# zivy/LSQRRecipes

Hardware: AMD Instinct MI355X
Metric: RANSAC hypotheses/sec + final-fit residual, 10M pts, 1/2/4/8 GPU (higher is better)
Workload: dtype f64; 1 GPU; PlaneParametersEstimator + RANSAC, 10000000 points, 50% outliers, delta=0.50 (BASELINE.json configs[1]); points=10000000, streams=4, world_size=1, collectives=none (single GPU), repeats=3

## Files before the change

### include/lsqr_hip.h

```cpp
#ifndef LSQR_HIP_H
#define LSQR_HIP_H

#include <stddef.h>
#include <stdint.h>

#ifdef __cplusplus
extern "C" {
#endif

#if defined(__GNUC__)
#define LSQR_API __attribute__((visibility("default")))
#else
#define LSQR_API
#endif

typedef enum {
  LSQR_OK = 0,
  LSQR_EMPTY = 1,
  LSQR_ERR_INVALID = 2,
  LSQR_ERR_NO_DEVICE = 3,
  LSQR_ERR_HIP = 4,
  LSQR_ERR_STATE = 5
} lsqr_status;

// ... 218 lines not shown
LSQR_API int lsqr_multi_upload(lsqr_multi *m, const void *host_records, size_t count, size_t stride_bytes);
LSQR_API int lsqr_multi_batch_fit(lsqr_multi *m, uint64_t seed, uint64_t first_index, size_t H_per_device,
                                  double *params_out, uint8_t *consensus_out, lsqr_ransac_info *info);
LSQR_API int lsqr_multi_ransac(lsqr_multi *m, double p, uint64_t seed, double *params_out,
                               uint8_t *consensus_out, lsqr_ransac_info *info);

LSQR_API int lsqr_ransac_exhaustive(lsqr_ctx *ctx, double *params_out, uint8_t *consensus_out,
                                    lsqr_ransac_info *info);
LSQR_API int lsqr_replay_init(size_t n, int k, double p, uint64_t state[6]);
LSQR_API size_t lsqr_replay(size_t n, int k, double p, const uint32_t *subsets,
                            const uint8_t *valid, const uint32_t *votes, size_t H,
                            uint64_t base_index, void *dedup_set, uint64_t state[6]);
LSQR_API void *lsqr_dedup_create(int k);
LSQR_API void lsqr_dedup_destroy(void *set);

LSQR_API int lsqr_set_option(lsqr_ctx *ctx, const char *name, int value);

LSQR_API int lsqr_index_info(const lsqr_ctx *ctx, uint64_t out[4]);

LSQR_API int lsqr_scan_workload(lsqr_ctx *ctx, uint32_t *bound_out, uint64_t out[8]);

LSQR_API int lsqr_scan_work(lsqr_ctx *ctx, uint64_t out[8]);

LSQR_API int lsqr_lm_persist_info(const lsqr_ctx *ctx, uint64_t out[8], uint64_t *trace, uint32_t trace_cap,
                                  uint32_t *trace_n);

LSQR_API int lsqr_profile_enable(lsqr_ctx *ctx, int on);
LSQR_API int lsqr_profile_get(lsqr_ctx *ctx, int kernel_id, uint64_t *launches, double *total_ms);
LSQR_API int lsqr_profile_reset(lsqr_ctx *ctx);

#ifdef __cplusplus
}
#endif
#endif
```

### lsqrrecipes_amd/_lib.py

```python
import ctypes as C
import os

import numpy as np

_HERE = os.path.dirname(os.path.abspath(__file__))
LIB_PATH = os.path.join(_HERE, "liblsqr_hip.so")

OK, EMPTY, ERR_INVALID, ERR_NO_DEVICE, ERR_HIP, ERR_STATE = range(6)
PLANE, SPHERE, LINE, DENSE, US_SINGLE, US_POINTER, ABSOR, PIVOT, RAY, LINE2D, PHANTOM = 1, 2, 3, 4, 5, 6, 7, 8, 9, 10, 11
LS_ALGEBRAIC, LS_GEOMETRIC = 0, 1
LS_ANALYTIC, LS_ITERATIVE = 0, 1
KERNEL_IDS = {"sample": 0, "estimate": 1, "scan": 2, "mask": 3, "moments": 4, "solve": 5,
              "index": 6, "absmax": 7}


class LsqrError(RuntimeError):
    def __init__(self, status, msg):
        RuntimeError.__init__(self, "lsqr_hip status %d: %s" % (status, msg))
        self.status = status


class ModelCfg(C.Structure):
    _fields_ = [("model", C.c_int32), ("dim", C.c_int32), ("delta", C.c_double),
                ("ls_type", C.c_int32), ("reserved", C.c_int32), ("aux", C.c_double)]
# ... 110 lines not shown
    "lsqr_batch_fit_wait": (C.c_int, [_ctx, C.c_int, C.c_void_p, C.POINTER(RansacInfo)]),
    "lsqr_multi_create": (C.c_int, [C.POINTER(C.c_int), C.c_int, C.POINTER(C.c_void_p)]),
    "lsqr_multi_destroy": (None, [C.c_void_p]),
    "lsqr_multi_size": (C.c_int, [C.c_void_p]),
    "lsqr_multi_transport": (C.c_char_p, [C.c_void_p, C.POINTER(C.c_double)]),
    "lsqr_multi_ctx": (C.c_void_p, [C.c_void_p, C.c_int]),
    "lsqr_multi_last_error": (C.c_char_p, [C.c_void_p]),
    "lsqr_multi_set_model": (C.c_int, [C.c_void_p, C.POINTER(ModelCfg)]),
    "lsqr_multi_upload": (C.c_int, [C.c_void_p, C.c_void_p, C.c_size_t, C.c_size_t]),
    "lsqr_multi_batch_fit": (C.c_int, [C.c_void_p, C.c_uint64, C.c_uint64, C.c_size_t, C.c_void_p, C.c_void_p,
                                       C.POINTER(RansacInfo)]),
    "lsqr_multi_ransac": (C.c_int, [C.c_void_p, C.c_double, C.c_uint64, C.c_void_p, C.c_void_p,
                                    C.POINTER(RansacInfo)]),
    "lsqr_ransac_exhaustive": (C.c_int, [_ctx, C.c_void_p, C.c_void_p, C.POINTER(RansacInfo)]),
    "lsqr_replay_init": (C.c_int, [C.c_size_t, C.c_int, C.c_double, _u64p]),
    "lsqr_replay": (C.c_size_t, [C.c_size_t, C.c_int, C.c_double, C.c_void_p, C.c_void_p,
                                 C.c_void_p, C.c_size_t, C.c_uint64, C.c_void_p, _u64p]),
    "lsqr_dedup_create": (C.c_void_p, [C.c_int]),
    "lsqr_dedup_destroy": (None, [C.c_void_p]),
    "lsqr_set_option": (C.c_int, [_ctx, C.c_char_p, C.c_int]),
    "lsqr_index_info": (C.c_int, [_ctx, _u64p]),
    "lsqr_scan_workload": (C.c_int, [_ctx, C.c_void_p, _u64p]),
    "lsqr_scan_work": (C.c_int, [_ctx, _u64p]),
    "lsqr_lm_persist_info": (C.c_int, [_ctx, _u64p, _u64p, C.c_uint32, C.POINTER(C.c_uint32)]),
    "lsqr_profile_enable": (C.c_int, [_ctx, C.c_int]),
    "lsqr_profile_get": (C.c_int, [_ctx, C.c_int, _u64p, _dp]),
    "lsqr_profile_reset": (C.c_int, [_ctx]),
}

_lib = None


def load():
    global _lib
    if _lib is None:
        if not os.path.exists(LIB_PATH):
            raise LsqrError(ERR_NO_DEVICE, "%s not built: run `python -c 'import __graft_entry__ as"
                            " g; g.build()'` or make -C lsqrrecipes_amd/csrc" % LIB_PATH)
        lib = C.CDLL(LIB_PATH)
        for name, (res, args) in SIGNATURES.items():
            fn = getattr(lib, name)
            fn.restype = res
            fn.argtypes = args
        _lib = lib
    return _lib

# ... 10 lines not shown
```

### lsqrrecipes_amd/context.py

```python
import ctypes as C

import numpy as np

from . import _lib as L


class Context:
    def __init__(self, device=0):
        self._lib = L.load()
        h = C.c_void_p()
        st = self._lib.lsqr_ctx_create(int(device), C.byref(h))
        if st != L.OK:
            raise L.LsqrError(st, "lsqr_ctx_create(device=%d): %s" % (
                device, self._lib.lsqr_status_string(st).decode()))
        self._h = h
        self.device = device
        self.cfg = None
        self._keep = None

    def close(self):
        if getattr(self, "_h", None):
            self._lib.lsqr_ctx_destroy(self._h)
            self._h = None

# ... 663 lines not shown
        self._chk(self._lib.lsqr_index_info(self._h, out))
        return {"built": bool(out[0]), "observations": int(out[1]), "cells": int(out[2]),
                "cell_points": int(out[3])}

    def scan_workload(self, want_bounds=False):
        H = self._lib.lsqr_num_hypotheses(self._h)
        ub = np.zeros(H, dtype=np.uint32) if want_bounds else None
        out = (C.c_uint64 * 8)()
        self._chk(self._lib.lsqr_scan_workload(self._h, L.ptr(ub), out))
        r = {"pairs": int(out[0]), "level1_evaluations": int(out[1]), "cells": int(out[2]),
             "cell_points": int(out[3]), "bounded": bool(out[4]), "pilots": int(out[5]),
             "second_pass": int(out[6]), "pairs_counted": int(out[7])}
        if want_bounds:
            r["bounds"] = ub
        return r

    def scan_work(self):
        out = (C.c_uint64 * 8)()
        self._chk(self._lib.lsqr_scan_work(self._h, out))
        return {"early_exit": bool(out[0]), "row_hypothesis_pairs": int(out[1]), "row_hypothesis_pairs_all": int(out[2]),
                "candidates": int(out[3]), "dropped_first": int(out[4]), "alive_at_end": int(out[5]),
                "ambiguous_pairs": int(out[6]), "band_records": int(out[7])}

    def synchronize(self):
        self._chk(self._lib.lsqr_synchronize(self._h))


class MultiContext:

    def __init__(self, devices):
        self._lib = L.load()
        arr = (C.c_int * len(devices))(*[int(d) for d in devices])
        h = C.c_void_p()
        st = self._lib.lsqr_multi_create(arr, len(devices), C.byref(h))
        if st != L.OK:
            raise L.LsqrError(st, "lsqr_multi_create(%s): %s" % (list(devices), self._lib.lsqr_status_string(st).decode()))
        self._h = h
        self.size = len(devices)
        self.cfg = None

    def close(self):
        if getattr(self, "_h", None):
            self._lib.lsqr_multi_destroy(self._h)
            self._h = None

    __del__ = close
# ... 91 lines not shown
```

### lsqrrecipes_amd/csrc/axis.h

```cpp
#pragma once
#include <hip/hip_runtime.h>
#include <stdint.h>

#include "cells.h"

namespace lsqr {

struct CellAxis {
  float e[3];
  float tmax;
};
constexpr int kAxisGroup = 8;

template <int NPT>
__global__ __launch_bounds__(256) void k_cell_moments(const double *__restrict__ sorted, size_t ns, uint32_t ncells,
                                                      const CellBox *__restrict__ boxes, double *__restrict__ mom) {
  const uint32_t cell = blockIdx.x * 4 + (threadIdx.x >> 6);
  if (cell >= ncells) return;
  const int lane = threadIdx.x & 63;
  constexpr uint32_t CP = 64 * NPT;
  const CellBox bx = boxes[cell];
  double s[10] = {0, 0, 0, 0, 0, 0, 0, 0, 0, 0};
  for (int k = 0; k < NPT; k++) {
    const size_t i = (size_t)cell * CP + k * 64 + lane;
// ... 124 lines not shown
  bool ok[NPT];
#pragma unroll
  for (int k = 0; k < NPT; k++) {
    const unsigned long long v = s[k * 64 + lane];
    const uint32_t src = (uint32_t)(v & 0xFFFFFFFFu), key = (uint32_t)(v >> 32);
    ok[k] = key != 0xFFFFFFFFu;
    const size_t i = (size_t)cell * CP + (ok[k] ? src : 0);
    const size_t ic = i < ns ? i : 0;
    px[k] = sorted[ic * 3], py[k] = sorted[ic * 3 + 1], pz[k] = sorted[ic * 3 + 2];
    uint32_t u = key;
    u ^= (u >> 31) ? 0x80000000u : 0xFFFFFFFFu;
    tv[k] = ok[k] ? __builtin_bit_cast(float, u) : __builtin_inff();
  }
  asm volatile("s_waitcnt vmcnt(0)" ::: "memory");
  __syncthreads();
  if (!live) return;
#pragma unroll
  for (int k = 0; k < NPT; k++) {
    const size_t i = (size_t)cell * CP + k * 64 + lane;
    cellT[i] = tv[k];
    if (ok[k] && i < ns) sorted[i * 3] = px[k], sorted[i * 3 + 1] = py[k], sorted[i * 3 + 2] = pz[k];
  }
  if (lane == 0) axis[cell].tmax = tmax;
}

template <int PP>
__global__ __launch_bounds__(512) void k_bound_axis(const CellBox *__restrict__ boxes, const CellAxis *__restrict__ axis,
                                                    const float *__restrict__ cellT, size_t ns, uint32_t ncells,
                                                    const float *__restrict__ rows, uint32_t H,
                                                    const uint32_t *__restrict__ h_dev, CellConsts cc, float thr_up,
                                                    float thr_dn, float xabs, uint32_t cells_per_block,
                                                    uint32_t *__restrict__ ub, uint32_t *__restrict__ lb) {
  typedef PlaneCell<3> CM;
  constexpr uint32_t CP = 128 * PP;
  constexpr int ROW = CM::ROW, NR4 = ROW / 4;
  const int lane = threadIdx.x & 63;
  if (h_dev) {
    const uint32_t hd = *h_dev;
    H = hd < H ? hd : H;
  }
  const uint32_t grp = blockIdx.y * 8 + (threadIdx.x >> 6);
  const uint32_t h = grp * 64 + lane;
  if (blockIdx.y * 512 >= H) return;
  const bool active = h - lane < H;
  float row[ROW];
  {
// ... 184 lines not shown
```

### lsqrrecipes_amd/csrc/cells.h

```cpp
#pragma once
#include <hip/hip_runtime.h>
#include <stdint.h>

#include "models.h"

#pragma clang diagnostic ignored "-Winline-asm"

namespace lsqr {

constexpr int kCellPtsMin = 128;
constexpr uint32_t kGroupPad = 4, kCellPad = 16;
constexpr uint32_t kBlockPad = 6;
constexpr uint32_t kQueues = 32;
constexpr uint32_t kQueuePitch = 1088;

struct CellBox {
  float c[3];
  float h[3];
  float pad[2];
};

__device__ inline unsigned long long ord_u64(double v) {
  unsigned long long b;
  __builtin_memcpy(&b, &v, 8);
  return (b >> 63) ? ~b : (b | 0x8000000000000000ULL);
}
inline double ord_u64_inv(unsigned long long o) {
  unsigned long long b = (o >> 63) ? (o & 0x7FFFFFFFFFFFFFFFULL) : ~o;
  double v;
  memcpy(&v, &b, 8);
  return v;
}

struct BoundsRow {
  unsigned long long mn[3], mx[3], amax, nonfinite;
};
template <int D>
__global__ __launch_bounds__(256) void k_bounds(const double *__restrict__ data, size_t stride,
                                                size_t n, BoundsRow *__restrict__ rows) {
  unsigned long long mn[D], mx[D], am = 0, bad = 0;
  for (int d = 0; d < D; d++) mn[d] = ~0ULL, mx[d] = 0ULL;
  auto one = [&](const double(&x)[D]) {
// ... 539 lines not shown
      sb.c[d] = cf;
      sb.h[d] = (!nan && hd <= 3.4e38) ? f32_up(hd) : 3.4028234e38f;
      r2 += (double)sb.h[d] * (double)sb.h[d];
    } else {
      sb.c[d] = 0.0f;
      sb.h[d] = 0.0f;
    }
  }
  const double rad = sqrt(r2) * (1.0 + 1e-6);
  sb.pad[0] = rad <= 3.4e38 ? f32_up(rad) : 3.4028234e38f;
  sb.pad[1] = 0.0f;
  sboxes[sc] = sb;
}

struct CellConsts {
  float f[8];
};
template <class CM>
constexpr bool cell_prepared() {
  if constexpr (requires { CM::PREPARED; }) return CM::PREPARED != 0;
  return false;
}
template <class CM>
struct HypWords {
  static_assert(sizeof(typename CM::Hyp) % 16 == 0, "a prepared Hyp is padded to a multiple of 16 bytes");
  enum { N4 = sizeof(typename CM::Hyp) / 16 };
  float w[4 * N4];
};
__device__ inline double f64_from(const float *w) {
  const unsigned long long bits = (unsigned long long)__builtin_bit_cast(uint32_t, w[0]) |
                                  ((unsigned long long)__builtin_bit_cast(uint32_t, w[1]) << 32);
  return __builtin_bit_cast(double, bits);
}

template <int D>
struct PlaneCell {
  typedef PlaneModel<D> M;
  enum { NB = 6, NV = 4, RELATIVE = 1, ROW = 4 * D, ROW_F32 = 0, ROW2 = 0, ROW2_OFF = 0 };
  enum { DEFAULT_CELL = 512, LDS_BROADCAST = 0, MIN_WAVES = 6 };
  enum { LDS_BROADCAST_PAIRS = 1 };
  enum { FULL_COUNT_PAIRS = 1 };
  enum { USE_BOUND = 1 };
  enum { BOUND_MERGE = 4 };
  struct Hyp {
    double n[3], c;
    float nf[3], e0;
  };
  enum { PREPARED = 1 };
  static __device__ inline void load(const float *row, const float *row2, bool valid,
                                     const CellConsts &cc, Hyp &h) {
    prepare(row, row2, valid, cc, h);
  }
  static __device__ inline void prepare(const float *row, const float *, bool valid,
                                        const CellConsts &cc, Hyp &h) {
    double r[2 * D];
#pragma unroll
    for (int i = 0; i < 2 * D; i++) r[i] = f64_from(row + 2 * i);
    bool ok = true;
    h.c = 0.0;
#pragma unroll
    for (int i = 0; i < 3; i++) {
      const double ni = i < D ? (valid ? r[i] : __builtin_nan("")) : 0.0;
      h.n[i] = ni;
      h.nf[i] = (float)ni;
      if (i < D) {
        h.c += ni * r[D + i];
        ok = ok && fabs(ni) <= 1.0000001;
      }
    }
    h.e0 = ok ? cc.f[2] : __builtin_inff();
  }
  static __device__ inline bool level1(const Hyp &h, const CellBox &b, const double *ctr,
                                       const CellConsts &cc, float *bc) {
    double d = -h.c;
    float rr = 0.0f;
#pragma unroll
    for (int i = D - 1; i >= 0; i--) {
      d = fma(h.n[i], ctr[i], d);
      rr = __builtin_fmaf(__builtin_fabsf(h.nf[i]), b.h[i], rr);
    }
    const float d0 = (float)d;
    const float E = __builtin_fmaf(rr, cc.f[3], h.e0);
    const float tout = (cc.f[1] + E) * 1.0000003f;
    const float tin = (cc.f[0] - E) * 0.9999997f;
    bc[0] = h.nf[0], bc[1] = h.nf[1], bc[2] = h.nf[2], bc[3] = d0, bc[4] = tin, bc[5] = tout;
    return __builtin_fabsf(d0) < (rr + tout) * 1.000004f;
  }
  static __device__ inline v2f value(const v2f *xs, const v2f *fp) {
    v2f s = fp[3];
    if (D == 3) s = __builtin_elementwise_fma(xs[2], fp[2], s);
    s = __builtin_elementwise_fma(xs[1], fp[1], s);
    s = __builtin_elementwise_fma(xs[0], fp[0], s);
    return s;
  }
};

inline float f32_up_host(double v) {
  float f = (float)v;
  if ((double)f < v) f = nextafterf(f, INFINITY);
  return f;
}
inline float f32_down_host(double v) {
  float f = (float)v;
  if ((double)f > v) f = nextafterf(f, -INFINITY);
  return f;
}
template <int D>
inline CellConsts cell_consts(const PlaneCell<D> *, const ModelConsts &mc) {
  const double u = 5.9604644775390625e-08;
// ... 687 lines not shown
#pragma unroll
  for (int k = 0; k < NH4; k++)
    out[(size_t)h * NH4 + k] = make_float4(hw.w[4 * k], hw.w[4 * k + 1], hw.w[4 * k + 2], hw.w[4 * k + 3]);
}
template <class CM>
__device__ __forceinline__ typename CM::Hyp hyp_from(const float4 (&v)[HypWords<CM>::N4]) {
  HypWords<CM> hw;
#pragma unroll
  for (int k = 0; k < HypWords<CM>::N4; k++)
    hw.w[4 * k] = v[k].x, hw.w[4 * k + 1] = v[k].y, hw.w[4 * k + 2] = v[k].z, hw.w[4 * k + 3] = v[k].w;
  return __builtin_bit_cast(typename CM::Hyp, hw);
}

template <class Box, class Store>
__device__ __forceinline__ void bounds_chunk(const CellBox *s_box, const double (*s_ctr)[3], const uint32_t n, Box &&box,
                                             Store &&store) {
  uint32_t i = 0;
  for (; i + 4 <= n; i += 4) {
    const CellBox b0 = s_box[i], b1 = s_box[i + 1], b2 = s_box[i + 2], b3 = s_box[i + 3];
    const double t0[3] = {s_ctr[i][0], s_ctr[i][1], s_ctr[i][2]};
    const double t1[3] = {s_ctr[i + 1][0], s_ctr[i + 1][1], s_ctr[i + 1][2]};
    const double t2[3] = {s_ctr[i + 2][0], s_ctr[i + 2][1], s_ctr[i + 2][2]};
    const double t3[3] = {s_ctr[i + 3][0], s_ctr[i + 3][1], s_ctr[i + 3][2]};
    const auto r0 = box(b0, t0), r1 = box(b1, t1), r2 = box(b2, t2), r3 = box(b3, t3);
    store(r0, r1, r2, r3);
  }
  for (; i < n; i++) {
    const CellBox b0 = s_box[i];
    const double t0[3] = {s_ctr[i][0], s_ctr[i][1], s_ctr[i][2]};
    store(box(b0, t0));
  }
}
template <class T, class... R>
__device__ __forceinline__ T *bounds_put(T *p, const uint32_t gstride, const int lane, const R... r) {
  const T v[] = {r...};
  if (lane == 0) {
#pragma unroll
    for (uint32_t k = 0; k < (uint32_t)sizeof...(R); k++) p[k * gstride] = v[k];
  }
  return p + (uint32_t)sizeof...(R) * gstride;
}
template <class CM, int PP, BoundsForm F>
__global__ __launch_bounds__(256) void k_cells_bounds(const CellBox *__restrict__ boxes, uint32_t ncells,
                                                      size_t ns, const float *__restrict__ rows,
                                                      const float *__restrict__ spf, uint32_t H,
                                                      CellConsts cc, uint32_t cells_per_block,
                                                      uint32_t *__restrict__ ub,
                                                      unsigned long long *__restrict__ total,
                                                      uint32_t *__restrict__ ncells_out,
                                                      uint8_t *__restrict__ cnt, uint32_t gstride,
                                                      const uint32_t *__restrict__ h_dev, uint32_t h_off,
                                                      uint32_t box_pop, const float4 *__restrict__ hyps) {
  static_assert(bounds_form_exists<CM, F>());
  constexpr bool PREP = prepared(F), COUNT = count(F), MASK = mask(F);
  typedef typename CM::M M;
  constexpr int ROW = CM::ROW, NR4 = ROW / 4, NR2 = CM::ROW2 / 4;
  const size_t CP = box_pop;
  const int lane = threadIdx.x & 63;
  if (h_dev) {
    const uint32_t hd = *h_dev > h_off ? *h_dev - h_off : 0u;
    H = hd < H ? hd : H;
  }
  const uint32_t grp = COUNT ? blockIdx.y * 4 + (uint32_t)__builtin_amdgcn_readfirstlane((int)(threadIdx.x >> 6))
                             : blockIdx.y * 4 + (threadIdx.x >> 6);
  const uint32_t h = grp * 64 + lane;
  if (blockIdx.y * 256 >= H) return;
  const bool active = h - lane < H;
  typename CM::Hyp hy;
  if constexpr (PREP) {
    constexpr int NH4 = HypWords<CM>::N4;
    float4 v[NH4];
#pragma unroll
    for (int k = 0; k < NH4; k++) v[k] = hyps[(size_t)(active ? h : 0) * NH4 + k];
    hy = hyp_from<CM>(v);
  } else {
    float row[ROW], row2[NR2 ? 4 * NR2 : 4];
    {
      const float4 *r4 = (const float4 *)(rows + (size_t)(h < H ? h : 0) * ROW);
#pragma unroll
      for (int k = 0; k < NR4; k++) {
        const float4 v = r4[k];
        row[4 * k] = v.x, row[4 * k + 1] = v.y, row[4 * k + 2] = v.z, row[4 * k + 3] = v.w;
      }
      if constexpr (NR2 > 0) {
        const float4 *q4 = (const float4 *)(spf + (size_t)(h < H ? h : 0) * M::SPF + CM::ROW2_OFF);
#pragma unroll
        for (int k = 0; k < NR2; k++) {
          const float4 v = q4[k];
          row2[4 * k] = v.x, row2[4 * k + 1] = v.y, row2[4 * k + 2] = v.z, row2[4 * k + 3] = v.w;
        }
      }
    }
    CM::load(row, row2, h < H, cc, hy);
  }
  const uint32_t c0 = blockIdx.x * cells_per_block;
  const uint32_t c1 = c0 + cells_per_block < ncells ? c0 + cells_per_block : ncells;
  uint32_t u = 0, nc = 0;
  constexpr uint32_t BCH = 128;
  __shared__ CellBox s_box[BCH];
  __shared__ double s_ctr[BCH][3];
  for (uint32_t cb = c0; cb < c1; cb += BCH) {
    const uint32_t n = c1 - cb < BCH ? c1 - cb : BCH;
    __syncthreads();
    if (threadIdx.x < 2 * n) ((float4 *)s_box)[threadIdx.x] = ((const float4 *)(boxes + cb))[threadIdx.x];
    __syncthreads();
    if (threadIdx.x < n) {
#pragma unroll
      for (int d = 0; d < 3; d++) s_ctr[threadIdx.x][d] = (double)s_box[threadIdx.x].c[d];
    }
    __syncthreads();
    if (!active) continue;
    if constexpr (MASK) {
      unsigned long long *p = (unsigned long long *)cnt + ((size_t)cb * gstride + grp);
      bounds_chunk(
          s_box, s_ctr, n,
          [&](const CellBox &bx, const double(&ctr)[3]) {
            float bc[CM::NB];
            return (unsigned long long)__ballot(CM::level1(hy, bx, ctr, cc, bc));
          },
          [&](auto... m) { p = bounds_put(p, gstride, lane, m...); });
    } else if constexpr (COUNT) {
      uint8_t *p = cnt + ((size_t)cb * gstride + grp);
      bounds_chunk(
          s_box, s_ctr, n,
          [&](const CellBox &bx, const double(&ctr)[3]) {
            float bc[CM::NB];
            const uint32_t pc = (uint32_t)__builtin_popcountll(__ballot(CM::level1(hy, bx, ctr, cc, bc)));
            return (uint8_t)(pc ? pc + kGroupPad : 0u);
          },
          [&](auto... pc) { p = bounds_put(p, gstride, lane, pc...); });
    } else {
      auto one = [&](const uint32_t i, const CellBox &bx, const double (&ctr)[3]) {
        const uint32_t c = cb + i;
        float bc[CM::NB];
        const bool s = CM::level1(hy, bx, ctr, cc, bc);
        const size_t first = (size_t)c * CP;
        const uint32_t pop = first + CP <= ns ? (uint32_t)CP : (uint32_t)(ns - first);
        u += s ? pop : 0u;
        nc += s ? 1u : 0u;
        if (cnt) {
          const uint32_t pc = (uint32_t)__builtin_popcountll(__ballot(s));
          if (lane == 0) cnt[(size_t)c * gstride + grp] = (uint8_t)(pc ? pc + kGroupPad : 0u);
        }
      };
      uint32_t i = 0;
      for (; i + 4 <= n; i += 4) {
        const CellBox b0 = s_box[i], b1 = s_box[i + 1], b2 = s_box[i + 2], b3 = s_box[i + 3];
        const double t0[3] = {s_ctr[i][0], s_ctr[i][1], s_ctr[i][2]};
// ... 66 lines not shown
                        __builtin_popcount(v.w));
      }
    for (; g < G; g++) t += (uint32_t)__builtin_popcountll(p[g]);
    t = pack_cell_cost(t);
    cost[c] = t;
  } else if (c < ncells) {
    const uint8_t *p = cnt + (size_t)c * gstride;
    uint32_t g = 0;
    if ((gstride & 15u) == 0)
      for (; g + 16 <= G; g += 16) {
        const uint4 v = *(const uint4 *)(p + g);
        t += __builtin_amdgcn_sad_u8(v.x, 0u, 0u) + __builtin_amdgcn_sad_u8(v.y, 0u, 0u) +
             __builtin_amdgcn_sad_u8(v.z, 0u, 0u) + __builtin_amdgcn_sad_u8(v.w, 0u, 0u);
      }
    for (; g < G; g++) t += p[g];
    t = t ? t + kCellPad : 0u;
    cost[c] = t;
  }
  __shared__ uint32_t s_w[2];
  for (int o = 32; o > 0; o >>= 1) t += __shfl_down(t, o);
  if ((threadIdx.x & 63) == 0) s_w[threadIdx.x >> 6] = t;
  __syncthreads();
  if (threadIdx.x == 0) csum[blockIdx.x] = s_w[0] + s_w[1];
}

__device__ __forceinline__ uint32_t wave_incl_scan(uint32_t v, int lane) {
#pragma unroll
  for (int o = 1; o < 64; o <<= 1) {
    const uint32_t a = __shfl_up(v, o);
    v += lane >= o ? a : 0u;
  }
  return v;
}

__device__ __forceinline__ uint32_t wave_incl_scan_dpp(uint32_t v) {
  v += (uint32_t)__builtin_amdgcn_update_dpp(0, (int)v, 0x111, 0xf, 0xf, false);
  v += (uint32_t)__builtin_amdgcn_update_dpp(0, (int)v, 0x112, 0xf, 0xf, false);
  v += (uint32_t)__builtin_amdgcn_update_dpp(0, (int)v, 0x114, 0xf, 0xf, false);
  v += (uint32_t)__builtin_amdgcn_update_dpp(0, (int)v, 0x118, 0xf, 0xf, false);
  v += (uint32_t)__builtin_amdgcn_update_dpp(0, (int)v, 0x142, 0xa, 0xf, false);
  v += (uint32_t)__builtin_amdgcn_update_dpp(0, (int)v, 0x143, 0xc, 0xf, false);
  return v;
}

struct PairsWave {
  const double *sorted;
// ... 433 lines not shown
```

### lsqrrecipes_amd/csrc/lsqr_hip.hip

```cpp
#include <hip/hip_runtime.h>

#include <algorithm>
#include <atomic>
#include <chrono>
#include <cmath>
#include <cstdarg>
#include <cstddef>
#include <cstdio>
#include <cstdlib>
#include <cstring>
#include <limits>
#include <set>
#include <thread>
#include <string>
#include <type_traits>
#include <utility>
#include <vector>

#include "../../include/lsqr_hip.h"
#include "devbuf.h"
#include "kernels.h"
#include "models_nd.h"
#include "dense.h"
#include "dense_h16.h"
// ... 147 lines not shown
  Us16Scales us16_sc{};
  int opt_us_h16 = 1;
  int opt_dense_fast = 1;
  int opt_us_fast = 1;
  DevBuf<uint8_t> d_refused;
  int opt_phantom_fast = 1;
  int opt_lm_tiles = 1;
  int opt_us_mask_mfma = 1;
  int opt_refine = 1;
  int opt_kd_levels = 7;
  int opt_kd_after = 16384;
  int kd_build_levels = 0, index_kd_levels = 0;
  int opt_presorted = 0;
  int opt_dense_wave = 3;
  int opt_dense_dd = 1;
  DevBuf<double> d_ddpart;
  int opt_index = 1, opt_cpt = 0, opt_cell = 0, opt_block = 0, opt_hsplit = 0, opt_pairs = 0, opt_pairs_waves = 0;
  DevBuf<uint8_t> d_valid;
  DevBuf<uint32_t> d_votes;
  DevBuf<uint32_t> d_ub;
  DevBuf<CellAxis> d_axis;
  DevBuf<float> d_cellT;
  bool axis_valid = false;
  int opt_mom_chunk = 0;
  int opt_hyp_order = 1;
  int opt_axis = 1;
  DevBuf<uint32_t> d_ub2;
  DevBuf<uint8_t> d_paircnt;
  DevBuf<uint32_t> d_paircost;
  DevBuf<uint32_t> d_vpart;
  DevBuf<float4> d_hyps;
  int opt_lean = 1;
  DevBuf<unsigned long long> d_pairmask;
  int opt_pack = 1;
  int opt_recheck = 1;
  DevBuf<unsigned long long> d_ambcnt;
  bool amb_reset = false;
  bool amb_counted = false;
  int opt_prepared = 1;
  DevBuf<uint32_t> d_sel;
  DevBuf<BoundSel> d_bsel;
  DevBuf<double> d_hparams2;
  DevBuf<float> d_hparams2_f32;
  DevBuf<uint32_t> d_votes2;
  int opt_bound = 1;
  uint32_t best_before = 0;
// ... 433 lines not shown
};
template <int D>
struct CellOf<LineModel<D>> {
  typedef LineCell<D> type;
};

void lanes_quiesce(lsqr_ctx *c) {
  for (int i = 1; i < lsqr_ctx::kMaxLanes; i++)
    if (c->lanes[i]) {
      (void)hipStreamSynchronize(c->lanes[i]->stream);
      for (int s = 0; s < 2; s++) c->lanes[i]->slot_busy[s] = false;
    }
}

void drop_index(lsqr_ctx *c) {
  c->h16_valid = false;
  c->us16_valid = false;
  c->h16_nomem = c->us16_nomem = false;
  c->n_sorted = 0;
  c->n_cells = 0;
  c->index_valid = false;
  c->index_kd_levels = 0;
  c->axis_valid = false;
}

template <int D>
int run_bounds(lsqr_ctx *c) {
  if (c->bounds_valid) return LSQR_OK;
  const int nb = grid_for(c->n, 256 * 16, 1024);
  BoundsRow *rows = (BoundsRow *)c->d_partials.get();
  static_assert(sizeof(BoundsRow) == 64, "BoundsRow is 8 words");
  {
    ProfScope ps(c, KID_ABSMAX);
    hipLaunchKernelGGL((k_bounds<D>), dim3(nb), dim3(256), 0, c->stream, c->d_data, c->stride, c->n, rows);
  }
  HIPCHK(c, hipGetLastError());
  hipLaunchKernelGGL(k_bounds_final, dim3(1), dim3(256), 0, c->stream, rows, nb, rows + 1024);
  HIPCHK(c, hipGetLastError());
  HIPCHK(c, hipMemcpyAsync(c->h_pin->scratch, rows + 1024, sizeof(BoundsRow), hipMemcpyDeviceToHost, c->stream));
  HIPCHK(c, sync_stream(c));
  memcpy(&c->h_bounds, c->h_pin->scratch, sizeof(BoundsRow));
  c->bounds_valid = true;
  return LSQR_OK;
}

template <int D>
// ... 95 lines not shown
      IDXCHK(sort_pairs_u32(tmp, &tmp_bytes, k_in, k_out, q_b, q_a, n, 16u + segbits, c->stream));
    }
    if (any) {
      hipLaunchKernelGGL(k_seg_compose, dim3(gn), dim3(256), 0, c->stream, v_out, q_a, n, q_b);
      IDXCHK(hipGetLastError());
      perm = q_b;
    }
    (void)hipFuncSetAttribute((const void *)k_refine_runs<D>, hipFuncAttributeMaxDynamicSharedMemorySize,
                              (int)refine_lds_bytes(D));
    const unsigned runs = (unsigned)((n_sorted + kRunPts - 1) / kRunPts);
    hipLaunchKernelGGL((k_refine_runs<D>), dim3(runs), dim3(1024), refine_lds_bytes(D), c->stream, c->d_data, c->stride,
                       perm, n_sorted, cell_pts);
    IDXCHK(hipGetLastError());
  }
  if (c->n_cells) {
    hipLaunchKernelGGL((k_gather_boxes<D>), dim3((c->n_cells + 3) / 4), dim3(256), 0, c->stream, c->d_data,
                       c->stride, perm, c->n_sorted, c->n_cells, cell_pts, c->d_sorted, c->d_boxes);
    IDXCHK(hipGetLastError());
  }
  c->axis_valid = false;
  if (D == 3 && c->opt_axis && c->cfg.model == LSQR_MODEL_PLANE && c->n_cells && (cell_pts == 512 || cell_pts == 256)) {
    if ((st = ensure(c, c->d_axis, (size_t)c->n_cells)) != LSQR_OK) return st;
    if ((st = ensure(c, c->d_cellT, (size_t)c->n_cells * cell_pts)) != LSQR_OK) return st;
    double *d_cmom = (double *)c->d_idx_scratch.get();
    if ((size_t)c->n_cells * 10 * sizeof(double) <= c->d_idx_scratch.cap()) {
      const unsigned gc = (c->n_cells + 3) / 4;
      if (cell_pts == 512) {
        hipLaunchKernelGGL((k_cell_moments<8>), dim3(gc), dim3(256), 0, c->stream, c->d_sorted, c->n_sorted, c->n_cells,
                           c->d_boxes, d_cmom);
      } else {
        hipLaunchKernelGGL((k_cell_moments<4>), dim3(gc), dim3(256), 0, c->stream, c->d_sorted, c->n_sorted, c->n_cells,
                           c->d_boxes, d_cmom);
      }
      const unsigned ngrp = (c->n_cells + kAxisGroup - 1) / kAxisGroup;
      hipLaunchKernelGGL(k_cell_axes, dim3((ngrp + 255) / 256), dim3(256), 0, c->stream, d_cmom, c->d_boxes, c->n_cells,
                         c->d_axis);
      if (cell_pts == 512)
        hipLaunchKernelGGL((k_cell_sort<8>), dim3(gc), dim3(256), 0, c->stream, c->d_sorted, c->n_sorted, c->n_cells,
                           c->d_boxes, c->d_axis, c->d_cellT);
      else
        hipLaunchKernelGGL((k_cell_sort<4>), dim3(gc), dim3(256), 0, c->stream, c->d_sorted, c->n_sorted, c->n_cells,
                           c->d_boxes, c->d_axis, c->d_cellT);
      IDXCHK(hipGetLastError());
      c->axis_valid = true;
    }
  }
#undef IDXCHK
  c->index_kd_levels = c->kd_build_levels;
  c->index_valid = true;
  return LSQR_OK;
}

struct ScanBatch {
  const double *sp;
  const float *spf;
  size_t H;
  uint32_t *votes;
  const uint32_t *h_dev;
  uint32_t h_off = 0;
};

template <class CM, int PP, int CPT, int BS, bool LDSB = false>
int launch_scan_cells(lsqr_ctx *c, const ScanBatch &b) {
  typedef typename CM::M M;
  const CellConsts cc = cell_consts((const CM *)nullptr, c->mc);
// ... 70 lines not shown
  }
  if (d_nc || merge < 2 || c->n_cells < 4 * merge) merge = 1;
  const CellBox *boxes = c->d_boxes;
  uint32_t nbox = c->n_cells;
  if (merge > 1) {
    nbox = (c->n_cells + merge - 1) / merge;
    if (c->super_merge != merge) {
      hipLaunchKernelGGL((k_super_boxes<M::ND>), dim3((nbox + 255) / 256), dim3(256), 0, c->stream, c->d_boxes,
                         c->n_cells, c->d_boxes + c->n_cells, nbox, merge);
      HIPCHK(c, hipGetLastError());
      c->super_merge = merge;
    }
    boxes = c->d_boxes + c->n_cells;
  }
  const unsigned gy = (unsigned)((c->H + 255) / 256);
  unsigned gx = std::max(1u, std::min<unsigned>(nbox, 2048u / gy));
  const uint32_t per = (nbox + gx - 1) / gx;
  gx = (nbox + per - 1) / per;
  hipLaunchKernelGGL((k_cells_bounds<CM, PP, BoundsForm::General>), dim3(gx, gy), dim3(256), 0, c->stream, boxes, nbox,
                     c->n_sorted,
                     CM::ROW_F32 ? c->d_hparams_f32 : (const float *)c->d_hparams.get(), c->d_hparams_f32,
                     (uint32_t)c->H, cc, per, d_ub, d_nc ? c->d_counter + CNT_PAIRS : (unsigned long long *)nullptr, d_nc,
                     (uint8_t *)nullptr, 0u, (const uint32_t *)nullptr, 0u,
                     (uint32_t)(128 * PP) * merge, (const float4 *)nullptr);
  HIPCHK(c, hipGetLastError());
  return LSQR_OK;
}

template <class CM>
PairsForm pairs_form(bool ldsb, bool opt_prepared, bool opt_lean, bool opt_pack, bool opt_recheck) {
  if (!cell_prepared<CM>() || !opt_prepared) return PairsForm::General;
  if (!opt_lean) return PairsForm::Prepared;
  if (!opt_pack) return PairsForm::Lean;
  const bool can_recheck = ldsb && pairs_form_exists<CM, true, PairsForm::PackedRecheck>();
  return can_recheck && opt_recheck ? PairsForm::PackedRecheck : PairsForm::Packed;
}
template <class CM, class F>
int with_pairs_form(PairsForm form, bool ldsb, F &&f) {
  auto go = [&](auto fc) { return ldsb ? f(fc, std::true_type{}) : f(fc, std::false_type{}); };
  if constexpr (cell_prepared<CM>()) {
    if constexpr (pairs_form_exists<CM, true, PairsForm::PackedRecheck>()) {
      if (form == PairsForm::PackedRecheck && ldsb)
        return f(std::integral_constant<PairsForm, PairsForm::PackedRecheck>{}, std::true_type{});
    }
    if (form == PairsForm::Packed) return go(std::integral_constant<PairsForm, PairsForm::Packed>{});
    if (form == PairsForm::Lean) return go(std::integral_constant<PairsForm, PairsForm::Lean>{});
    if (form == PairsForm::Prepared) return go(std::integral_constant<PairsForm, PairsForm::Prepared>{});
// ... 35 lines not shown
  const PairsForm form = pairs_form<CM>(ldsb, c->opt_prepared, c->opt_lean, c->opt_pack, c->opt_recheck);
  if constexpr (cell_prepared<CM>()) {
    if (prepared(form)) {
      const uint32_t slots = (Hc + 63) & ~63u;
      if ((st = ensure(c, c->d_hyps, (size_t)slots * HypWords<CM>::N4)) != LSQR_OK) return st;
      hipLaunchKernelGGL((k_prepare_hyps<CM>), dim3((slots + 255) / 256), dim3(256), 0, c->stream, rows, b.spf, Hc, cc,
                         b.h_dev, b.h_off, c->d_hyps);
      HIPCHK(c, hipGetLastError());
    }
  }
  const float4 *hyps = prepared(form) ? c->d_hyps : nullptr;
  if (packed(form) && (st = ensure(c, c->d_pairmask, (size_t)c->n_cells * gstride)) != LSQR_OK) return st;
  uint8_t *d_cnt = packed(form) ? (uint8_t *)c->d_pairmask.get() : c->d_paircnt.get();
  constexpr int BS = 256, wpb = BS / 64;
  const size_t lds = (size_t)((Hc + 3) & ~3u) * sizeof(uint32_t) + (ldsb ? (size_t)wpb * 2048 : 0) +
                     (packed(form) ? (size_t)wpb * 256 : 0);
  return with_pairs_form<CM>(form, ldsb, [&](auto form_c, auto ldsb_c) -> int {
    constexpr PairsForm F = decltype(form_c)::value;
    constexpr bool LDSB = decltype(ldsb_c)::value;
    {
      const unsigned gy = (Hc + 255) / 256;
      const uint32_t per = std::max<uint32_t>(8, (c->n_cells + 1023) / 1024);
      const unsigned gx = (c->n_cells + per - 1) / per;
      auto count = [&](auto kern) {
        hipLaunchKernelGGL(kern, dim3(gx, gy), dim3(256), 0, c->stream, c->d_boxes, c->n_cells, c->n_sorted, rows, b.spf,
                           Hc, cc, per, (uint32_t *)nullptr, (unsigned long long *)nullptr, (uint32_t *)nullptr,
                           d_cnt, gstride, b.h_dev, b.h_off, (uint32_t)(128 * PP), hyps);
      };
      if (c->opt_lean)
        count(k_cells_bounds<CM, PP, bounds_form(F, true)>);
      else
        count(k_cells_bounds<CM, PP, bounds_form(F, false)>);
      HIPCHK(c, hipGetLastError());
    }
    hipLaunchKernelGGL(k_tile_costs<packed(F)>, dim3(nchunks), dim3(kChunkCells), 0, c->stream, (const uint8_t *)d_cnt,
                       gstride, Hc, b.h_dev, c->n_cells, d_cost, d_csum, b.votes, b.h_off,
                       c->amb_reset ? c->d_ambcnt.get() : (unsigned long long *)nullptr);
    c->amb_reset = false;
    c->amb_counted = cell_prepared<CM>() && M::ND == 3;
    HIPCHK(c, hipGetLastError());
    const auto kern = k_scan_pairs<CM, PP, BS, LDSB, F>;
    int per_cu = (int)std::min<size_t>(32 / wpb, (160 * 1024) / std::max<size_t>(lds, 1)), occ = 0;
    if (hipOccupancyMaxActiveBlocksPerMultiprocessor(&occ, kern, BS, lds) == hipSuccess && occ >= 1)
      per_cu = std::min(per_cu, occ);
    else
      (void)hipGetLastError();
    if (per_cu < 1) per_cu = 1;
    if (c->opt_pairs_waves > 0) per_cu = std::min(per_cu, c->opt_pairs_waves);
    const unsigned blocks = (unsigned)std::min<size_t>(((size_t)c->n_cells + wpb - 1) / wpb, (size_t)256 * per_cu);
    int st2 = ensure(c, c->d_vpart, (size_t)blocks * Hc);
// ... 723 lines not shown
    return run_scan_f32<M, 4, 1>(c);
  }
  if (ppl == 8) return run_scan_f32<M, 8>(c);
  if (ppl == 16) return run_scan_f32<M, 16>(c);
  return run_scan_f32<M, 4>(c);
}
template <class M>
int scan_exact(lsqr_ctx *c) {
  if constexpr (M::REC <= 3) {
    int ppl = c->opt_ppl ? c->opt_ppl : 8;
    if (ppl == 2) return run_scan_ppl<M, 2>(c);
    if (ppl == 8) return run_scan_ppl<M, 8>(c);
    return run_scan_ppl<M, 4>(c);
  } else {
    return run_scan_ppl<M, M::PPL>(c);
  }
}

int run_scan(lsqr_ctx *c) {
  c->hyp_since_upload += c->H;
  c->ee_last = false;
  c->amb_reset = true;
  c->amb_counted = false;
  return dispatch(c->cfg, [&](auto tag) -> int {
    typedef typename decltype(tag)::type M;
    bool done = false;
    int st = LSQR_OK;
    if constexpr (M::IS_DENSE) st = scan_dense<M>(c, &done);
    if (st != LSQR_OK || done) return st;
    if constexpr (requires { M::NF32; }) {
      st = scan_us<M>(c, &done);
    } else if constexpr (requires { M::SPF; }) {
      if constexpr (requires { typename CellOf<M>::type; }) st = scan_indexed<M>(c, &done);
      if (st == LSQR_OK && !done) st = scan_f32<M>(c, &done);
    }
    if (st != LSQR_OK || done) return st;
    return scan_exact<M>(c);
  });
}

int run_scan_batch(lsqr_ctx *c, uint32_t best_before) {
  c->allow_bound = true;
  c->best_before = best_before;
  int st = run_scan(c);
  c->allow_bound = false;
  c->best_before = 0;
// ... 3182 lines not shown
  }
  if (!strcmp(name, "scan_pairs")) {
    c->opt_pairs = value;
    return LSQR_OK;
  }
  if (!strcmp(name, "scan_prepared")) {
    c->opt_prepared = value != 0;
    return LSQR_OK;
  }
  if (!strcmp(name, "scan_lean")) {
    c->opt_lean = value != 0;
    return LSQR_OK;
  }
  if (!strcmp(name, "scan_pack")) {
    if (value != 0 && value != 1) return fail(c, LSQR_ERR_INVALID, "scan_pack must be 0 or 1");
    c->opt_pack = value;
    return LSQR_OK;
  }
  if (!strcmp(name, "scan_recheck")) {
    if (value != 0 && value != 1) return fail(c, LSQR_ERR_INVALID, "scan_recheck must be 0 or 1");
    c->opt_recheck = value;
    return LSQR_OK;
  }
  if (!strcmp(name, "scan_axis")) {
    c->opt_axis = value != 0;
    return LSQR_OK;
  }
  if (!strcmp(name, "scan_hyp_order")) {
    c->opt_hyp_order = value != 0;
    return LSQR_OK;
  }
  if (!strcmp(name, "mom_chunk")) {
    c->opt_mom_chunk = value;
    return LSQR_OK;
  }
  if (!strcmp(name, "us_mfma")) {
    c->opt_us_h16 = value != 0;
    return LSQR_OK;
  }
  if (!strcmp(name, "scan_pairs_mfma")) {
    return value == 0 ? LSQR_OK : fail(c, LSQR_ERR_INVALID, "scan_pairs_mfma: removed (measured slower; tools/attic/cells_h16.h)");
  }
  if (!strcmp(name, "scan_pairs_waves")) {
    c->opt_pairs_waves = value;
    return LSQR_OK;
  }
// ... 184 lines not shown
  if (c->amb_counted)
    HIPCHK(c, hipMemcpyAsync(pin, c->d_ambcnt, 2 * kAmbSlots * sizeof(unsigned long long), hipMemcpyDeviceToHost, c->stream));
  HIPCHK(c, sync_stream(c));
  const uint64_t all = (uint64_t)c->H * (uint64_t)c->n;
  memset(out, 0, 8 * sizeof(uint64_t));
  if (c->amb_counted)
    for (int k = 0; k < kAmbSlots; k++) out[6] += pin[2 * k], out[7] += pin[2 * k + 1];
  out[2] = all;
  if (c->ee_last && c->h_ee && c->ee_H == c->H && c->ee_n == c->n) {
    out[0] = 1;
    out[1] = c->h_ee->work;
    out[3] = c->h_ee->n_cand;
    out[4] = c->h_ee->n_drop_first;
    out[5] = c->h_ee->n_alive;
  } else {
    out[1] = all;
    bsel_host_synced(c);
    if (c->last_bound[0] && c->last_bound[3] == c->H && c->bsel_known_H == c->H)
      out[3] = c->bsel_known.n_cand;
  }
  return LSQR_OK;
}

int lsqr_index_info(const lsqr_ctx *c, uint64_t out[4]) {
  if (!c || !out) return LSQR_ERR_INVALID;
  out[0] = c->index_valid ? 1 : 0;
  out[1] = c->n_sorted;
  out[2] = c->n_cells;
  out[3] = c->cell_pts;
  return LSQR_OK;
}

int lsqr_profile_enable(lsqr_ctx *c, int on) {
  if (!c) return LSQR_ERR_INVALID;
  prof_flush(c);
  c->prof = on != 0;
  for (int i = 1; i < lsqr_ctx::kMaxLanes; i++)
    if (c->lanes[i]) lsqr_profile_enable(c->lanes[i], on);
  return LSQR_OK;
}
int lsqr_profile_get(lsqr_ctx *c, int id, uint64_t *launches, double *total_ms) {
  if (!c || id < 0 || id >= 8) return LSQR_ERR_INVALID;
  prof_flush(c);
  uint64_t n = c->launches[id];
  double ms = c->ms[id];
  for (int i = 1; i < lsqr_ctx::kMaxLanes; i++)
// ... 23 lines not shown
```

Baseline: 7.002 million hypotheses/s.

## Add per-cell axis slab test to prune hypothesis-cell pairs in masked bounds

Adds a per-cell slab record built from each cell's principal axis and sorted projection range. The masked bounds kernel uses it as a second, tighter plane-vs-cell rejection test after the box test, so fewer hypothesis-cell pairs survive into the exact scan. This costs an extra kernel at index build, LDS staging of the slabs, and extra ALU work per surviving pair. A diagnostic API for counting surviving pairs is also added.

```diff
diff --git a/include/lsqr_hip.h b/include/lsqr_hip.h
--- a/include/lsqr_hip.h
+++ b/include/lsqr_hip.h
@@ -264,6 +264,8 @@
 
 LSQR_API int lsqr_scan_work(lsqr_ctx *ctx, uint64_t out[8]);
 
+LSQR_API int lsqr_scan_pairs_counted(lsqr_ctx *ctx, uint64_t out[4]);
+
 LSQR_API int lsqr_lm_persist_info(const lsqr_ctx *ctx, uint64_t out[8], uint64_t *trace, uint32_t trace_cap,
                                   uint32_t *trace_n);
 
diff --git a/lsqrrecipes_amd/_lib.py b/lsqrrecipes_amd/_lib.py
--- a/lsqrrecipes_amd/_lib.py
+++ b/lsqrrecipes_amd/_lib.py
@@ -156,6 +156,7 @@
     "lsqr_index_info": (C.c_int, [_ctx, _u64p]),
     "lsqr_scan_workload": (C.c_int, [_ctx, C.c_void_p, _u64p]),
     "lsqr_scan_work": (C.c_int, [_ctx, _u64p]),
+    "lsqr_scan_pairs_counted": (C.c_int, [_ctx, _u64p]),
     "lsqr_lm_persist_info": (C.c_int, [_ctx, _u64p, _u64p, C.c_uint32, C.POINTER(C.c_uint32)]),
     "lsqr_profile_enable": (C.c_int, [_ctx, C.c_int]),
     "lsqr_profile_get": (C.c_int, [_ctx, C.c_int, _u64p, _dp]),
diff --git a/lsqrrecipes_amd/context.py b/lsqrrecipes_amd/context.py
--- a/lsqrrecipes_amd/context.py
+++ b/lsqrrecipes_amd/context.py
@@ -709,6 +709,11 @@
                 "candidates": int(out[3]), "dropped_first": int(out[4]), "alive_at_end": int(out[5]),
                 "ambiguous_pairs": int(out[6]), "band_records": int(out[7])}
 
+    def scan_pairs_counted(self):
+        out = (C.c_uint64 * 4)()
+        self._chk(self._lib.lsqr_scan_pairs_counted(self._h, out))
+        return {"pairs": int(out[0]), "masks": bool(out[1]), "slab": bool(out[2]), "table_entries": int(out[3])}
+
     def synchronize(self):
         self._chk(self._lib.lsqr_synchronize(self._h))
 
diff --git a/lsqrrecipes_amd/csrc/axis.h b/lsqrrecipes_amd/csrc/axis.h
--- a/lsqrrecipes_amd/csrc/axis.h
+++ b/lsqrrecipes_amd/csrc/axis.h
@@ -170,6 +170,39 @@
     if (ok[k] && i < ns) sorted[i * 3] = px[k], sorted[i * 3 + 1] = py[k], sorted[i * 3 + 2] = pz[k];
   }
   if (lane == 0) axis[cell].tmax = tmax;
+}
+
+__global__ __launch_bounds__(256) void k_cell_slabs(const CellBox *__restrict__ boxes, const CellAxis *__restrict__ axis,
+                                                    const float *__restrict__ cellT, size_t ns, uint32_t ncells,
+                                                    uint32_t cell_pts, double xabs, uint32_t gate4,
+                                                    CellSlab *__restrict__ slabs) {
+  const uint32_t c = blockIdx.x * 256 + threadIdx.x;
+  if (c >= ncells) return;
+  const CellBox bx = boxes[c];
+  const CellAxis ax = axis[c];
+  const size_t first = (size_t)c * cell_pts;
+  const uint32_t pop = first >= ns ? 0u : (first + cell_pts <= ns ? cell_pts : (uint32_t)(ns - first));
+  CellSlab s;
+  const double e0 = (double)ax.e[0], e1 = (double)ax.e[1], e2 = (double)ax.e[2], ee = e0 * e0 + e1 * e1 + e2 * e2;
+  const double r1 = (double)bx.h[0] + (double)bx.h[1] + (double)bx.h[2];
+  s.e[0] = ax.e[0], s.e[1] = ax.e[1], s.e[2] = ax.e[2];
+  s.iee = (float)(1.0 / ee);
+  s.tmid = 0.0f, s.tspan = __builtin_inff(), s.pad = 0.0f;
+  const double eabs = (1.3e-7 * r1 + 4e-12 * xabs) * (1.0 + 1e-6);
+  s.eabs = eabs <= 3.4e38 ? f32_up(eabs) : __builtin_inff();
+  if (pop) {
+    const double t0 = (double)cellT[first], t1 = (double)cellT[first + pop - 1];
+    const double lo = t0 - (6e-8 * fabs(t0) + 2e-13 * xabs), hi = t1 + (6e-8 * fabs(t1) + 2e-13 * xabs);
+    const float mid = (float)(0.5 * lo + 0.5 * hi);
+    const double span = fmax(hi - (double)mid, (double)mid - lo) * (1.0 + 1e-12);
+    const double box_e = fabs(e0) * (double)bx.h[0] + fabs(e1) * (double)bx.h[1] + fabs(e2) * (double)bx.h[2];
+    if (span >= 0.0 && span <= 1e30 && fabsf(mid) <= 1e30f && r1 <= 1e30 && ee > 0.25 && ee <= 4.0 &&
+        span * ee * 4.0 <= (double)gate4 * box_e) {
+      s.tmid = mid;
+      s.tspan = f32_up(span);
+    }
+  }
+  slabs[c] = s;
 }
 
 template <int PP>
diff --git a/lsqrrecipes_amd/csrc/cells.h b/lsqrrecipes_amd/csrc/cells.h
--- a/lsqrrecipes_amd/csrc/cells.h
+++ b/lsqrrecipes_amd/csrc/cells.h
@@ -18,6 +18,13 @@
   float c[3];
   float h[3];
   float pad[2];
+};
+struct CellSlab {
+  float e[3];
+  float iee;
+  float tmid, tspan;
+  float eabs;
+  float pad;
 };
 
 __device__ inline unsigned long long ord_u64(double v) {
@@ -603,6 +610,11 @@
   return false;
 }
 template <class CM>
+constexpr bool cell_slab() {
+  if constexpr (requires { CM::SLAB; }) return CM::SLAB != 0;
+  return false;
+}
+template <class CM>
 struct HypWords {
   static_assert(sizeof(typename CM::Hyp) % 16 == 0, "a prepared Hyp is padded to a multiple of 16 bytes");
   enum { N4 = sizeof(typename CM::Hyp) / 16 };
@@ -628,6 +640,7 @@
     float nf[3], e0;
   };
   enum { PREPARED = 1 };
+  enum { SLAB = D == 3 };
   static __device__ inline void load(const float *row, const float *row2, bool valid,
                                      const CellConsts &cc, Hyp &h) {
     prepare(row, row2, valid, cc, h);
@@ -666,6 +679,18 @@
     const float tin = (cc.f[0] - E) * 0.9999997f;
     bc[0] = h.nf[0], bc[1] = h.nf[1], bc[2] = h.nf[2], bc[3] = d0, bc[4] = tin, bc[5] = tout;
     return __builtin_fabsf(d0) < (rr + tout) * 1.000004f;
+  }
+  static __device__ inline bool slab(const Hyp &h, const float *bc, const CellBox &b, const CellSlab &s) {
+    static_assert(D == 3, "the axis-sorted index is built in 3-D");
+    const float al = __builtin_fmaf(h.nf[0], s.e[0], __builtin_fmaf(h.nf[1], s.e[1], h.nf[2] * s.e[2])) * s.iee;
+    const float m0 = __builtin_fmaf(-al, s.e[0], h.nf[0]), m1 = __builtin_fmaf(-al, s.e[1], h.nf[1]),
+                m2 = __builtin_fmaf(-al, s.e[2], h.nf[2]);
+    const float rho = __builtin_fmaf(__builtin_fabsf(m0), b.h[0],
+                                     __builtin_fmaf(__builtin_fabsf(m1), b.h[1], __builtin_fabsf(m2) * b.h[2]));
+    const float W = __builtin_fmaf(__builtin_fabsf(al), s.tspan, rho);
+    const float c = __builtin_fmaf(al, s.tmid, bc[3]);
+    const float r = __builtin_fmaf(1.000001f, W, bc[NB - 1]) + s.eabs;
+    return !(__builtin_fabsf(c) > r * 1.000001f);
   }
   static __device__ inline v2f value(const v2f *xs, const v2f *fp) {
     v2f s = fp[3];
@@ -1399,13 +1424,13 @@
     const double t1[3] = {s_ctr[i + 1][0], s_ctr[i + 1][1], s_ctr[i + 1][2]};
     const double t2[3] = {s_ctr[i + 2][0], s_ctr[i + 2][1], s_ctr[i + 2][2]};
     const double t3[3] = {s_ctr[i + 3][0], s_ctr[i + 3][1], s_ctr[i + 3][2]};
-    const auto r0 = box(b0, t0), r1 = box(b1, t1), r2 = box(b2, t2), r3 = box(b3, t3);
+    const auto r0 = box(i, b0, t0), r1 = box(i + 1, b1, t1), r2 = box(i + 2, b2, t2), r3 = box(i + 3, b3, t3);
     store(r0, r1, r2, r3);
   }
   for (; i < n; i++) {
     const CellBox b0 = s_box[i];
     const double t0[3] = {s_ctr[i][0], s_ctr[i][1], s_ctr[i][2]};
-    store(box(b0, t0));
+    store(box(i, b0, t0));
   }
 }
 template <class T, class... R>
@@ -1416,6 +1441,15 @@
     for (uint32_t k = 0; k < (uint32_t)sizeof...(R); k++) p[k * gstride] = v[k];
   }
   return p + (uint32_t)sizeof...(R) * gstride;
+}
+template <bool ON>
+__device__ __forceinline__ CellSlab *slab_lds() {
+  if constexpr (ON) {
+    __shared__ CellSlab s_slab[128];
+    return s_slab;
+  } else {
+    return nullptr;
+  }
 }
 template <class CM, int PP, BoundsForm F>
 __global__ __launch_bounds__(256) void k_cells_bounds(const CellBox *__restrict__ boxes, uint32_t ncells,
@@ -1427,9 +1461,11 @@
                                                       uint32_t *__restrict__ ncells_out,
                                                       uint8_t *__restrict__ cnt, uint32_t gstride,
                                                       const uint32_t *__restrict__ h_dev, uint32_t h_off,
-                                                      uint32_t box_pop, const float4 *__restrict__ hyps) {
+                                                      uint32_t box_pop, const float4 *__restrict__ hyps,
+                                                      const CellSlab *__restrict__ slabs) {
   static_assert(bounds_form_exists<CM, F>());
   constexpr bool PREP = prepared(F), COUNT = count(F), MASK = mask(F);
+  constexpr bool SLAB = MASK && cell_slab<CM>();
   typedef typename CM::M M;
   constexpr int ROW = CM::ROW, NR4 = ROW / 4, NR2 = CM::ROW2 / 4;
   const size_t CP = box_pop;
@@ -1474,12 +1510,16 @@
   const uint32_t c1 = c0 + cells_per_block < ncells ? c0 + cells_per_block : ncells;
   uint32_t u = 0, nc = 0;
   constexpr uint32_t BCH = 128;
+  static_assert(BCH == 128, "slab_lds() holds one chunk");
   __shared__ CellBox s_box[BCH];
   __shared__ double s_ctr[BCH][3];
   for (uint32_t cb = c0; cb < c1; cb += BCH) {
     const uint32_t n = c1 - cb < BCH ? c1 - cb : BCH;
     __syncthreads();
     if (threadIdx.x < 2 * n) ((float4 *)s_box)[threadIdx.x] = ((const float4 *)(boxes + cb))[threadIdx.x];
+    if constexpr (SLAB) {
+      if (slabs && threadIdx.x < 2 * n) ((float4 *)slab_lds<SLAB>())[threadIdx.x] = ((const float4 *)(slabs + cb))[threadIdx.x];
+    }
     __syncthreads();
     if (threadIdx.x < n) {
 #pragma unroll
@@ -1491,16 +1531,24 @@
       unsigned long long *p = (unsigned long long *)cnt + ((size_t)cb * gstride + grp);
       bounds_chunk(
           s_box, s_ctr, n,
-          [&](const CellBox &bx, const double(&ctr)[3]) {
+          [&](const uint32_t i, const CellBox &bx, const double(&ctr)[3]) {
             float bc[CM::NB];
-            return (unsigned long long)__ballot(CM::level1(hy, bx, ctr, cc, bc));
+            unsigned long long m = __ballot(CM::level1(hy, bx, ctr, cc, bc));
+            if constexpr (SLAB) {
+              if (slabs && m) {
+                const CellSlab sl = slab_lds<SLAB>()[i];
+                if (__builtin_amdgcn_readfirstlane(__builtin_bit_cast(int, sl.tspan)) < 0x7F800000)
+                  m &= __ballot(CM::slab(hy, bc, bx, sl));
+              }
+            }
+            return m;
           },
           [&](auto... m) { p = bounds_put(p, gstride, lane, m...); });
     } else if constexpr (COUNT) {
       uint8_t *p = cnt + ((size_t)cb * gstride + grp);
       bounds_chunk(
           s_box, s_ctr, n,
-          [&](const CellBox &bx, const double(&ctr)[3]) {
+          [&](const uint32_t, const CellBox &bx, const double(&ctr)[3]) {
             float bc[CM::NB];
             const uint32_t pc = (uint32_t)__builtin_popcountll(__ballot(CM::level1(hy, bx, ctr, cc, bc)));
             return (uint8_t)(pc ? pc + kGroupPad : 0u);
@@ -1613,6 +1661,40 @@
   if ((threadIdx.x & 63) == 0) s_w[threadIdx.x >> 6] = t;
   __syncthreads();
   if (threadIdx.x == 0) csum[blockIdx.x] = s_w[0] + s_w[1];
+}
+
+template <bool PACK>
+__global__ __launch_bounds__(1024) void k_pairs_in_table(const uint8_t *__restrict__ cnt, uint32_t gstride, uint32_t H,
+                                                         const uint32_t *__restrict__ h_dev, uint32_t h_off,
+                                                         uint32_t ncells, const uint32_t *__restrict__ cost,
+                                                         unsigned long long *__restrict__ out) {
+  unsigned long long t = 0;
+  if constexpr (PACK) {
+    for (uint32_t c = threadIdx.x; c < ncells; c += 1024) {
+      const uint32_t v = cost[c];
+      t += v ? pack_cell_survivors(v) : 0u;
+    }
+  } else {
+    if (h_dev) {
+      const uint32_t hd = *h_dev > h_off ? *h_dev - h_off : 0u;
+      H = hd < H ? hd : H;
+    }
+    const uint32_t G = (H + 63) / 64;
+    for (uint32_t c = threadIdx.x; c < ncells; c += 1024)
+      for (uint32_t g = 0; g < G; g++) {
+        const uint32_t b = cnt[(size_t)c * gstride + g];
+        t += b ? b - kGroupPad : 0u;
+      }
+  }
+  __shared__ unsigned long long s_t[16];
+  for (int o = 32; o > 0; o >>= 1) t += __shfl_down(t, o);
+  if ((threadIdx.x & 63) == 0) s_t[threadIdx.x >> 6] = t;
+  __syncthreads();
+  if (threadIdx.x == 0) {
+    unsigned long long a = 0;
+    for (int w = 0; w < 16; w++) a += s_t[w];
+    *out = a;
+  }
 }
 
 __device__ __forceinline__ uint32_t wave_incl_scan(uint32_t v, int lane) {
diff --git a/lsqrrecipes_amd/csrc/lsqr_hip.hip b/lsqrrecipes_amd/csrc/lsqr_hip.hip
--- a/lsqrrecipes_amd/csrc/lsqr_hip.hip
+++ b/lsqrrecipes_amd/csrc/lsqr_hip.hip
@@ -193,6 +193,14 @@
   DevBuf<CellAxis> d_axis;
   DevBuf<float> d_cellT;
   bool axis_valid = false;
+  DevBuf<CellSlab> d_slab;
+  int opt_slab = 1;
+  int opt_slab_gate = 3;
+  struct {
+    bool valid = false, packed = false, slab = false;
+    uint32_t H = 0, h_off = 0, gstride = 0;
+    const uint32_t *h_dev = nullptr;
+  } last_count;
   int opt_mom_chunk = 0;
   int opt_hyp_order = 1;
   int opt_axis = 1;
@@ -672,6 +680,7 @@
   c->index_valid = false;
   c->index_kd_levels = 0;
   c->axis_valid = false;
+  c->last_count.valid = false;
 }
 
 template <int D>
@@ -813,6 +822,7 @@
   if (D == 3 && c->opt_axis && c->cfg.model == LSQR_MODEL_PLANE && c->n_cells && (cell_pts == 512 || cell_pts == 256)) {
     if ((st = ensure(c, c->d_axis, (size_t)c->n_cells)) != LSQR_OK) return st;
     if ((st = ensure(c, c->d_cellT, (size_t)c->n_cells * cell_pts)) != LSQR_OK) return st;
+    if ((st = ensure(c, c->d_slab, (size_t)c->n_cells)) != LSQR_OK) return st;
     double *d_cmom = (double *)c->d_idx_scratch.get();
     if ((size_t)c->n_cells * 10 * sizeof(double) <= c->d_idx_scratch.cap()) {
       const unsigned gc = (c->n_cells + 3) / 4;
@@ -832,6 +842,12 @@
       else
         hipLaunchKernelGGL((k_cell_sort<4>), dim3(gc), dim3(256), 0, c->stream, c->d_sorted, c->n_sorted, c->n_cells,
                            c->d_boxes, c->d_axis, c->d_cellT);
+      {
+        double xabs;
+        memcpy(&xabs, &hb.amax, sizeof xabs);
+        hipLaunchKernelGGL(k_cell_slabs, dim3((c->n_cells + 255) / 256), dim3(256), 0, c->stream, c->d_boxes, c->d_axis,
+                           c->d_cellT, c->n_sorted, c->n_cells, cell_pts, xabs, (uint32_t)c->opt_slab_gate, c->d_slab);
+      }
       IDXCHK(hipGetLastError());
       c->axis_valid = true;
     }
@@ -948,7 +964,8 @@
                      CM::ROW_F32 ? c->d_hparams_f32 : (const float *)c->d_hparams.get(), c->d_hparams_f32,
                      (uint32_t)c->H, cc, per, d_ub, d_nc ? c->d_counter + CNT_PAIRS : (unsigned long long *)nullptr, d_nc,
                      (uint8_t *)nullptr, 0u, (const uint32_t *)nullptr, 0u,
-                     (uint32_t)(128 * PP) * merge, (const float4 *)nullptr);
+                     (uint32_t)(128 * PP) * merge, (const float4 *)nullptr,
+                     (const CellSlab *)nullptr);
   HIPCHK(c, hipGetLastError());
   return LSQR_OK;
 }
@@ -1030,10 +1047,16 @@
       const unsigned gy = (Hc + 255) / 256;
       const uint32_t per = std::max<uint32_t>(8, (c->n_cells + 1023) / 1024);
       const unsigned gx = (c->n_cells + per - 1) / per;
+      const CellSlab *slabs = nullptr;
+      if constexpr (packed(F) && cell_slab<CM>()) {
+        if (c->opt_slab && c->axis_valid && c->cell_pts == (uint32_t)(128 * PP)) slabs = c->d_slab;
+      }
+      c->last_count.valid = true, c->last_count.packed = packed(F), c->last_count.slab = slabs != nullptr;
+      c->last_count.H = Hc, c->last_count.h_off = b.h_off, c->last_count.gstride = gstride, c->last_count.h_dev = b.h_dev;
       auto count = [&](auto kern) {
         hipLaunchKernelGGL(kern, dim3(gx, gy), dim3(256), 0, c->stream, c->d_boxes, c->n_cells, c->n_sorted, rows, b.spf,
                            Hc, cc, per, (uint32_t *)nullptr, (unsigned long long *)nullptr, (uint32_t *)nullptr,
-                           d_cnt, gstride, b.h_dev, b.h_off, (uint32_t)(128 * PP), hyps);
+                           d_cnt, gstride, b.h_dev, b.h_off, (uint32_t)(128 * PP), hyps, slabs);
       };
       if (c->opt_lean)
         count(k_cells_bounds<CM, PP, bounds_form(F, true)>);
@@ -1803,6 +1826,7 @@
   c->ee_last = false;
   c->amb_reset = true;
   c->amb_counted = false;
+  c->last_count.valid = false;
   return dispatch(c->cfg, [&](auto tag) -> int {
     typedef typename decltype(tag)::type M;
     bool done = false;
@@ -5031,6 +5055,17 @@
     c->opt_recheck = value;
     return LSQR_OK;
   }
+  if (!strcmp(name, "scan_slab")) {
+    if (value != 0 && value != 1) return fail(c, LSQR_ERR_INVALID, "scan_slab must be 0 or 1");
+    c->opt_slab = value;
+    return LSQR_OK;
+  }
+  if (!strcmp(name, "scan_slab_gate")) {
+    if (value < 1 || value > 8) return fail(c, LSQR_ERR_INVALID, "scan_slab_gate must be 1..8 (quarters)");
+    c->opt_slab_gate = value;
+    drop_index(c);
+    return LSQR_OK;
+  }
   if (!strcmp(name, "scan_axis")) {
     c->opt_axis = value != 0;
     return LSQR_OK;
@@ -5261,6 +5296,31 @@
   return LSQR_OK;
 }
 
+int lsqr_scan_pairs_counted(lsqr_ctx *c, uint64_t out[4]) {
+  int st = need_ready(c, true);
+  if (st != LSQR_OK) return st;
+  if (!out) return fail(c, LSQR_ERR_INVALID, "null argument");
+  if (!c->scanned || !c->last_count.valid || !c->index_valid || c->n_cells == 0)
+    return fail(c, LSQR_ERR_STATE, "no counted scan over this index");
+  const auto &lc = c->last_count;
+  unsigned long long *d_sum = c->d_counter + CNT_SUM;
+  if (lc.packed)
+    hipLaunchKernelGGL(k_pairs_in_table<true>, dim3(1), dim3(1024), 0, c->stream, (const uint8_t *)nullptr, 0u, 0u,
+                       (const uint32_t *)nullptr, 0u, c->n_cells, (const uint32_t *)c->d_paircost.get(), d_sum);
+  else
+    hipLaunchKernelGGL(k_pairs_in_table<false>, dim3(1), dim3(1024), 0, c->stream, (const uint8_t *)c->d_paircnt.get(),
+                       lc.gstride, lc.H, lc.h_dev, lc.h_off, c->n_cells, (const uint32_t *)nullptr, d_sum);
+  HIPCHK(c, hipGetLastError());
+  unsigned long long *pin = c->h_pin->scratch_u64;
+  HIPCHK(c, hipMemcpyAsync(pin, d_sum, sizeof(unsigned long long), hipMemcpyDeviceToHost, c->stream));
+  HIPCHK(c, sync_stream(c));
+  out[0] = pin[0];
+  out[1] = lc.packed ? 1 : 0;
+  out[2] = lc.slab ? 1 : 0;
+  out[3] = (uint64_t)c->n_cells * lc.H;
+  return LSQR_OK;
+}
+
 int lsqr_index_info(const lsqr_ctx *c, uint64_t out[4]) {
   if (!c || !out) return LSQR_ERR_INVALID;
   out[0] = c->index_valid ? 1 : 0;
```

After: 7.524 million hypotheses/s (median of 6 runs). 7.5% higher.
